# Samirez/Visual_odometry

Hardware: AMD Instinct MI355X
Metric: frame-pairs/sec (1280x720, 2000 ORB feats) (higher is better)
Workload: dtype u8+f32+f64; 1 GPU; seeded synthetic 1280x720 drone flight (256 distinct rendered views, closed loop), 2000 ORB features/frame, 8 levels = BASELINE config 2; chunk of 257 consecutive frames -> 256 pairs (k, k+1) per GPU per step, each frame detected once; detector=orb, distinct_rendered_frames=256, pair_stride=1, contexts_per_gpu=3, keypoint_order=cv2, poly_solver=fast, matcher=crosscheck, matcher_kernel=mfma_fp4, ransac=5-point, conf 0.99, 1 px, seed 2^64-1, <=1000 iters, parallelism=single GPU, pairs_ok_last_step=256

## Files before the change

### include/vo_hip.h

```cpp
#ifndef VO_HIP_H
#define VO_HIP_H
#include <stddef.h>
#include <stdint.h>

#ifdef __cplusplus
extern "C" {
#endif

#define VO_MAX_LEVELS 16

#define VO_OK                 0
#define VO_WARN_CAPACITY      1
#define VO_ERR_INVALID       -1
#define VO_ERR_HIP           -2
#define VO_ERR_TOO_FEW       -3
#define VO_ERR_NO_MODEL      -4
#define VO_ERR_NOT_CONFIGURED -5
#define VO_ERR_UNSUPPORTED    -7
#define VO_ERR_AMBIGUOUS      -6

typedef struct vo_ctx vo_ctx;

typedef struct {
    int32_t nfeatures;
// ... 45 lines not shown

int vo_recover_pose(vo_ctx* ctx, const double* E, const double* p1, const double* p2, int M, const double* K,
                    double dist_thresh, double* R, double* t, uint8_t* mask, int32_t* n_good);

int vo_triangulate(vo_ctx* ctx, const double* P1, const double* P2, const double* x1, const double* x2,
                   int M, double* X);

int64_t vo_packed_pyramid_bytes(int h, int w, const vo_orb_params* params);
int vo_stage_pyramid(vo_ctx* ctx, const uint8_t* img, int h, int w, int channels, int row_stride,
                     const vo_orb_params* params, uint8_t* out_packed);
int vo_stage_fast_scores(vo_ctx* ctx, const uint8_t* img, int h, int w, int channels, int row_stride,
                         const vo_orb_params* params, uint8_t* out_packed);
int vo_stage_blur(vo_ctx* ctx, const uint8_t* img, int h, int w, int channels, int row_stride,
                  const vo_orb_params* params, uint8_t* out_packed);
int vo_stage_retain_best(vo_ctx* ctx, const float* response, int n, int n_points, int32_t* order, int32_t* n_out);
int vo_stage_five_point(vo_ctx* ctx, const double* x1, const double* x2, double* E , int32_t* n_models);

typedef struct {
    int32_t match_mode;
    double  ratio;
    double  ransac_prob;
    double  ransac_thresh;
    int32_t ransac_max_iters;
    uint64_t ransac_seed;
    double  pose_dist_thresh;
    int32_t want_points;
} vo_pair_opts;

typedef struct {
    int32_t n_kp1, n_kp2, n_match, n_inl, n_good, status, ransac_iters, reserved;
// ... 141 lines not shown
```

### visual_odometry_amd/_lib.py

```python
from __future__ import annotations

import ctypes as C
import os

import numpy as np

_HERE = os.path.dirname(os.path.abspath(__file__))
LIB_PATH = os.environ.get("VO_HIP_LIBRARY") or os.path.join(_HERE, "libvo_hip.so")

VO_OK, VO_WARN_CAPACITY = 0, 1
VO_ERR_INVALID, VO_ERR_HIP, VO_ERR_TOO_FEW, VO_ERR_NO_MODEL, VO_ERR_NOT_CONFIGURED, VO_ERR_AMBIGUOUS = -1, -2, -3, -4, -5, -6
VO_ERR_UNSUPPORTED = -7
VO_STAGE_COUNT = 28
VO_COMM_ID_BYTES, VO_RECORD_DOUBLES = 128, 16
VO_BA_MAX_CAMERAS, VO_BA_MAX_FREE = 64, 16


class OrbParams(C.Structure):
    _fields_ = [("nfeatures", C.c_int32), ("scale_factor", C.c_float), ("nlevels", C.c_int32),
                ("edge_threshold", C.c_int32), ("first_level", C.c_int32), ("wta_k", C.c_int32),
                ("score_type", C.c_int32), ("patch_size", C.c_int32), ("fast_threshold", C.c_int32)]


class SiftParams(C.Structure):
# ... 46 lines not shown
    "vo_frames_upload_color": (C.c_int, [_P, _P, C.c_int, C.c_int, C.c_int, C.c_int64, C.c_int]),
    "vo_frames_detect": (C.c_int, [_P, C.c_int, C.c_int]),
    "vo_frames_detect_async": (C.c_int, [_P, C.c_int, C.c_int]),
    "vo_batch_kp_capacity": (C.c_int, [_P]),
    "vo_host_alloc": (C.c_int, [C.c_size_t, C.POINTER(_P)]),
    "vo_host_free": (None, [_P]),
    "vo_frame_features": (C.c_int, [_P, C.c_int, _P, _P, _P, _P, _P, _P, C.c_int, _P]),
    "vo_pairs_run": (C.c_int, [_P, _P, C.c_int, _P, _P, _P, _P, C.c_int32]),
    "vo_pairs_run_async": (C.c_int, [_P, _P, C.c_int, _P, _P, _P, _P, C.c_int32]),
    "vo_sync": (C.c_int, [_P]),
    "vo_set_matcher_kernel": (C.c_int, [_P, C.c_int]),
    "vo_set_poly_solver": (C.c_int, [_P, C.c_int]),
    "vo_set_pnp_refine": (C.c_int, [_P, C.c_int]),
    "vo_set_keypoint_order": (C.c_int, [_P, C.c_int]),
    "vo_stage_retain_best": (C.c_int, [_P, _P, C.c_int, C.c_int, _P, _P]),
    "vo_detect_after": (C.c_int, [_P, _P]),
    "vo_knn2_hamming": (C.c_int, [_P, _P, C.c_int, _P, C.c_int, _P, _P]),
    "vo_knn2_l2": (C.c_int, [_P, _P, C.c_int, _P, C.c_int, C.c_int, _P, _P]),
    "vo_knn2_ratio_l2": (C.c_int, [_P, _P, C.c_int, _P, C.c_int, C.c_int, C.c_double, _P, _P, _P, _P]),
    "vo_tracks_pnp_batch": (C.c_int, [_P, C.c_int, _P, C.c_int, C.c_double, C.c_double, C.c_uint64, C.c_double, _P, _P, _P, _P, _P]),
    "vo_slam_chain": (C.c_int, [_P, C.c_int, _P, _P, _P, _P, _P, _P, _P, _P, _P, _P, _P, _P, _P]),
    "vo_slam_map_size": (C.c_int, [_P, C.c_int, _P, _P, _P]),
    "vo_slam_map": (C.c_int, [_P, C.c_int, _P, _P, _P, _P, _P, _P, _P, _P]),
    "vo_slam_chains": (C.c_int, [_P, C.c_int, _P, _P, _P, C.c_int, _P, _P, _P, _P, _P, _P, _P, _P, _P, _P, _P]),
    "vo_slam_chains_restart": (C.c_int, [_P, C.c_int, _P, _P, _P, C.c_int, _P, _P, _P, _P, _P, _P, _P, _P, _P, _P, _P, _P, _P, _P, _P]),
    "vo_slam_chains_map_size": (C.c_int, [_P, C.c_int, C.c_int, _P, _P, _P]),
    "vo_slam_chains_map": (C.c_int, [_P, C.c_int, C.c_int, _P, _P, _P, _P, _P, _P, _P, _P]),
    "vo_comm_unique_id": (C.c_int, [_P]),
    "vo_comm_init": (C.c_int, [_P, _P, C.c_int, C.c_int]),
    "vo_comm_destroy": (C.c_int, [_P]),
# ... 15 lines not shown
    "vo_batch_configure_sift": (C.c_int, [_P, C.c_int, C.c_int, _P, C.c_int, C.c_int, C.c_int]),
    "vo_frame_features_sift": (C.c_int, [_P, C.c_int, _P, _P, _P, _P, _P, _P, C.c_int, _P]),
    "vo_stage_sift_rows": (C.c_int, [_P, C.c_int, _P, C.c_int, _P]),
    "vo_jpeg_info": (C.c_int, [_P, C.c_size_t, _P, _P, _P, _P, _P]),
    "vo_jpeg_decode": (C.c_int, [_P, _P, C.c_size_t, _P, C.c_int, C.c_int, _P, _P]),
    "vo_jpeg_decode_batch": (C.c_int, [_P, _P, _P, C.c_int, _P, C.c_int, C.c_int]),
    "vo_frames_ingest_jpeg": (C.c_int, [_P, _P, _P, C.c_int, C.c_int, _P]),
    "vo_feature_tracks": (C.c_int, [_P, C.c_int, C.c_int, _P, _P, _P, _P, C.c_int, _P, _P, _P]),
    "vo_profile_enable": (C.c_int, [_P, C.c_int]),
    "vo_profile_reset": (C.c_int, [_P]),
    "vo_profile_read": (C.c_int, [_P, _P, _P]),
    "vo_stage_name": (C.c_char_p, [C.c_int]),
    "vo_stage_bytes": (C.c_double, [_P, C.c_int, C.c_int]),
}

_lib = None


def load():
    global _lib
    if _lib is not None:
        return _lib
    if not os.path.exists(LIB_PATH):
        raise ImportError(
            f"{LIB_PATH} not found: build the HIP library first (python -c 'import __graft_entry__ as g; g.build()' "
            "or make -C visual_odometry_amd/csrc). There is no CPU fallback.")
    lib = C.CDLL(LIB_PATH)
    for name, (res, args) in _SIGS.items():
        fn = getattr(lib, name)
        fn.restype = res
        fn.argtypes = args
    _lib = lib
    return lib


def exported_symbols():
    return sorted(_SIGS)


class VoError(RuntimeError):
    def __init__(self, code, msg):
        super().__init__(f"libvo_hip error {code}: {msg}")
        self.code = code
# ... 51 lines not shown

    def comm_info(self):
        n, r = C.c_int32(0), C.c_int32(0)
        self.check(self.lib.vo_comm_info(self.handle, C.addressof(n), C.addressof(r)))
        return n.value, r.value

    def allgather(self, values, world):
        v = np.ascontiguousarray(values, np.float64).ravel()
        out = np.empty((int(world), len(v)), np.float64)
        self.check(self.lib.vo_comm_allgather_f64(self.handle, v.ctypes.data, len(v), out.ctypes.data))
        return out

    def set_keypoint_order(self, kind):
        self.check(self.lib.vo_set_keypoint_order(self.handle, {"canonical": 0, "cv2": 1}[kind]))

    def retain_best(self, response, n_points):
        r = np.ascontiguousarray(response, np.float32)
        out = np.zeros(max(len(r), 1), np.int32)
        n = C.c_int32(0)
        self.check(self.lib.vo_stage_retain_best(self.handle, r.ctypes.data, len(r), int(n_points), out.ctypes.data, C.addressof(n)))
        return out[:n.value].copy()

    def set_poly_solver(self, kind):
        self.check(self.lib.vo_set_poly_solver(self.handle, {"fast": 0, "opencv300": 1}[kind]))

    def set_pnp_refine(self, kind):
        self.check(self.lib.vo_set_pnp_refine(self.handle, {"fast": 0, "cv2": 1}[kind]))

    def last_error(self) -> str:
        msg = self.lib.vo_last_error(self.handle)
        return msg.decode() if msg else ""

    def check(self, rc):
        if rc < 0:
            msg = self.lib.vo_last_error(self.handle)
# ... 61 lines not shown
```

### visual_odometry_amd/csrc/cv2order_kernels.hip

```cpp
#include "vo_internal.h"
#include <float.h>

#ifndef CV_THREADS
#define CV_THREADS 256
#endif
#ifndef CV_EPT
#define CV_EPT 4
#endif
#ifndef CV_LDS_CAP
#define CV_LDS_CAP 4096
#endif

__device__ __forceinline__ bool el_gt(uint2 x, uint2 y) { return __uint_as_float(x.x) > __uint_as_float(y.x); }

#define CV_TIE_CAP CV_THREADS
struct Cv2Shared {
    int cnt[2][CV_EPT][CV_THREADS / 64][2];
    int probe[2][CV_THREADS / 64];
    int ntie, nleft;
    uint32_t tie[CV_TIE_CAP], tie_sorted[CV_TIE_CAP], left[CV_TIE_CAP];
    uint8_t is_tie[CV_TIE_CAP];
};

__device__ __forceinline__ void rank2(const bool (&fl)[CV_EPT], const bool (&fr)[CV_EPT], int parity, Cv2Shared& sh,
                                      int (&rl)[CV_EPT], int (&rr)[CV_EPT], int& tl, int& tr)
{
    const int lane = threadIdx.x & 63, wave = threadIdx.x >> 6;
    const unsigned long long below = lane ? (~0ULL >> (64 - lane)) : 0ULL;
    unsigned long long ml[CV_EPT], mr[CV_EPT];
#pragma unroll
    for (int e = 0; e < CV_EPT; e++) {
        ml[e] = __ballot(fl[e]); mr[e] = __ballot(fr[e]);
        if (lane == 0) { sh.cnt[parity][e][wave][0] = (int)__popcll(ml[e]); sh.cnt[parity][e][wave][1] = (int)__popcll(mr[e]); }
    }
    __syncthreads();
    int sl = 0, sr = 0;
// ... 30 lines not shown
        if (lane == 0) sh.probe[par][wave] = m64 ? wave * 64 + (int)__ffsll((long long)m64) - 1 : CV_THREADS;
        __syncthreads();
        int tf = CV_THREADS;
#pragma unroll
        for (int w = 0; w < CV_THREADS / 64; w++) tf = min(tf, sh.probe[par][w]);
        par ^= 1;
        const int kt = lo + tf * step;
        const int nhi = tf < CV_THREADS && kt < hi ? kt : hi;
        const int nlo = tf > 0 ? min(lo + (tf - 1) * step + 1, nhi) : lo;
        lo = nlo; hi = nhi;
        if (step == 1) break;
    }
    return hi;
}

template <typename A>
__device__ void adjust_heap(A f, int hole, int len, uint2 v)
{
    const int top = hole;
    int sc = hole;
    while (sc < (len - 1) / 2) { sc = 2 * (sc + 1); if (el_gt(f[sc], f[sc - 1])) sc--; f[hole] = f[sc]; hole = sc; }
    if ((len & 1) == 0 && sc == (len - 2) / 2) { sc = 2 * (sc + 1); f[hole] = f[sc - 1]; hole = sc - 1; }
    int parent = (hole - 1) / 2;
    while (hole > top && el_gt(f[parent], v)) { f[hole] = f[parent]; hole = parent; parent = (hole - 1) / 2; }
    f[hole] = v;
}

template <typename A>
__device__ void heap_select(A a, int first, int middle, int last)
{
    A f = a + first;
    const int len = middle - first;
    if (len >= 2)
        for (int parent = (len - 2) / 2;; parent--) { const uint2 v = f[parent]; adjust_heap(f, parent, len, v); if (parent == 0) break; }
    for (int i = middle; i < last; i++)
        if (el_gt(a[i], a[first])) { const uint2 v = a[i]; a[i] = a[first]; adjust_heap(f, 0, len, v); }
}

template <typename A>
__device__ void insertion_sort(A a, int first, int last)
{
    if (first == last) return;
    for (int i = first + 1; i < last; i++) {
        const uint2 v = a[i];
        if (el_gt(v, a[first])) { for (int j = i; j > first; j--) a[j] = a[j - 1]; a[first] = v; }
        else { int nx = i - 1; while (el_gt(v, a[nx])) { a[nx + 1] = a[nx]; nx--; } a[nx + 1] = v; }
    }
}

template <int KIND, typename A, typename PosT>
__device__ __forceinline__ int partition_pass(A a, int first, int last, uint2 pivot, float thr, PosT* lpos, PosT* rpos, Cv2Shared& sh)
{
    const int tid = threadIdx.x;
    int nl = 0, nr = 0, parity = 0;
    const int begin = KIND == 0 ? first + 1 : first;
    for (int base = begin; base < last; base += CV_THREADS * CV_EPT, parity ^= 1) {
        bool fl[CV_EPT], fr[CV_EPT];
#pragma unroll
        for (int e = 0; e < CV_EPT; e++) {
            const int i = base + e * CV_THREADS + tid;
            fl[e] = fr[e] = false;
            if (i < last) {
                const uint2 v = a[i];
                if (KIND == 0) { fl[e] = !el_gt(v, pivot); fr[e] = !el_gt(pivot, v); }
                else { const bool pred = __uint_as_float(v.x) >= thr; fl[e] = !pred; fr[e] = pred; }
            }
        }
        int rl[CV_EPT], rr[CV_EPT], tl, tr;
        rank2(fl, fr, parity, sh, rl, rr, tl, tr);
#pragma unroll
        for (int e = 0; e < CV_EPT; e++) {
            const int i = base + e * CV_THREADS + tid;
            if (fl[e]) lpos[nl + rl[e]] = (PosT)i;
            if (fr[e]) rpos[nr + rr[e]] = (PosT)i;
        }
        nl += tl; nr += tr;
    }
    __syncthreads();
    int K;
    long long res;
    const long long INF = 1LL << 40;
    if (KIND == 0) {
        K = first_true_wg(min(nl, nr), sh, [&](int k) { return lpos[k] >= rpos[nr - 1 - k]; });
        const long long lk = K < nl ? (long long)lpos[K] : INF, rk = K > 0 ? (long long)rpos[nr - K] : INF;
        res = lk < rk ? lk : rk;
    } else {
        K = first_true_wg(nl, sh, [&](int k) { return k >= nr || lpos[k] > rpos[nr - 1 - k]; });
        if (K >= nl) res = K > 0 ? (long long)rpos[nr - K] : (long long)last;
        else if (K > 0 && lpos[K] > rpos[nr - K]) res = rpos[nr - K];
        else res = lpos[K];
    }
    for (int k = tid; k < K; k += CV_THREADS) {
        const int i = (int)lpos[k], j = (int)rpos[nr - 1 - k];
        const uint2 x = a[i], y = a[j];
        a[i] = y; a[j] = x;
    }
    __syncthreads();
    return (int)res;
}

template <typename A, typename PosT>
__device__ __forceinline__ int partition_pivot(A a, int first, int last, PosT* lpos, PosT* rpos, Cv2Shared& sh)
{
    if (threadIdx.x == 0) {
        const int Ai = first + 1, B = first + (last - first) / 2, C = last - 1;
        int m;
        if (el_gt(a[Ai], a[B])) m = el_gt(a[B], a[C]) ? B : el_gt(a[Ai], a[C]) ? C : Ai;
        else m = el_gt(a[Ai], a[C]) ? Ai : el_gt(a[B], a[C]) ? C : B;
        const uint2 t = a[first]; a[first] = a[m]; a[m] = t;
    }
    __syncthreads();
    const uint2 p = a[first];
    return partition_pass<0>(a, first, last, p, 0.f, lpos, rpos, sh);
}

template <typename A, typename PosT>
__device__ __forceinline__ void introselect_loop(A a, int& first, int& last, int nth, int& depth, bool& done, int stop, PosT* lpos, PosT* rpos, Cv2Shared& sh)
{
    while (last - first > stop) {
        if (last - first <= 3) break;
        if (depth == 0) {
            if (threadIdx.x == 0) { heap_select(a, first, nth + 1, last); const uint2 t = a[first]; a[first] = a[nth]; a[nth] = t; }
            __syncthreads();
            done = true;
            return;
        }
        depth--;
        const int cut = partition_pivot(a, first, last, lpos, rpos, sh);
        if (cut <= nth) first = cut; else last = cut;
    }
}

#ifndef CV_WAVE_CAP
#define CV_WAVE_CAP 256
#endif
#define CV_WSYNC() do { __builtin_amdgcn_fence(__ATOMIC_SEQ_CST, "wavefront"); __builtin_amdgcn_wave_barrier(); } while (0)
template <typename P>
// ... 3 lines not shown
    while (hi > lo) {
        const int step = (hi - lo + 63) / 64;
        const int k = lo + lane * step;
        const bool t = k < hi ? pred(k) : true;
        const unsigned long long m64 = __ballot(t);
        const int tf = m64 ? (int)__ffsll((long long)m64) - 1 : 64;
        const int kt = lo + tf * step;
        const int nhi = tf < 64 && kt < hi ? kt : hi;
        const int nlo = tf > 0 ? min(lo + (tf - 1) * step + 1, nhi) : lo;
        lo = nlo; hi = nhi;
        if (step == 1) break;
    }
    return hi;
}

__device__ __forceinline__ int partition_pivot_wave(uint2* a, int first, int last, uint16_t* lpos, uint16_t* rpos)
{
    const int lane = threadIdx.x & 63;
    if (lane == 0) {
        const int Ai = first + 1, B = first + (last - first) / 2, C = last - 1;
        int m;
        if (el_gt(a[Ai], a[B])) m = el_gt(a[B], a[C]) ? B : el_gt(a[Ai], a[C]) ? C : Ai;
        else m = el_gt(a[Ai], a[C]) ? Ai : el_gt(a[B], a[C]) ? C : B;
        const uint2 t = a[first]; a[first] = a[m]; a[m] = t;
    }
    CV_WSYNC();
    const uint2 pivot = a[first];
    const unsigned long long below = lane ? (~0ULL >> (64 - lane)) : 0ULL;
    int nl = 0, nr = 0;
    for (int base = first + 1; base < last; base += 64) {
        const int i = base + lane;
        bool fl = false, fr = false;
        if (i < last) { const uint2 v = a[i]; fl = !el_gt(v, pivot); fr = !el_gt(pivot, v); }
        const unsigned long long ml = __ballot(fl), mr = __ballot(fr);
        if (fl) lpos[nl + (int)__popcll(ml & below)] = (uint16_t)i;
        if (fr) rpos[nr + (int)__popcll(mr & below)] = (uint16_t)i;
        nl += (int)__popcll(ml); nr += (int)__popcll(mr);
    }
    CV_WSYNC();
    const int K = first_true_wave(min(nl, nr), lane, [&](int k) { return lpos[k] >= rpos[nr - 1 - k]; });
    const int INF = 1 << 30;
    const int lk = K < nl ? (int)lpos[K] : INF, rk = K > 0 ? (int)rpos[nr - K] : INF;
    for (int k = lane; k < K; k += 64) {
        const int i = (int)lpos[k], j = (int)rpos[nr - 1 - k];
        const uint2 x = a[i], y = a[j];
        a[i] = y; a[j] = x;
    }
    CV_WSYNC();
    return lk < rk ? lk : rk;
}

__device__ __forceinline__ void introselect_wave(uint2* a, int first, int last, int nth, int depth, uint16_t* lpos, uint16_t* rpos)
{
    const int lane = threadIdx.x & 63;
    while (last - first > 3) {
        if (depth == 0) {
            if (lane == 0) { heap_select(a, first, nth + 1, last); const uint2 t = a[first]; a[first] = a[nth]; a[nth] = t; }
            CV_WSYNC();
            return;
        }
        depth--;
        const int cut = partition_pivot_wave(a, first, last, lpos, rpos);
        if (cut <= nth) first = cut; else last = cut;
    }
    if (lane == 0) insertion_sort(a, first, last);
    CV_WSYNC();
}

template <typename A>
__device__ __forceinline__ int partition_ge_sparse(A a, int first, int last, float thr, Cv2Shared& sh)
{
    const int tid = threadIdx.x;
    if (tid == 0) sh.ntie = 0;
    __syncthreads();
    for (int i = first + tid; i < last; i += CV_THREADS)
        if (__uint_as_float(a[i].x) >= thr) { const int s = atomicAdd(&sh.ntie, 1); if (s < CV_TIE_CAP) sh.tie[s] = (uint32_t)i; }
    __syncthreads();
    const int nr = sh.ntie;
    if (nr > CV_TIE_CAP) return -1;
    if (nr == 0) return first;
    for (int i = tid; i < nr; i += CV_THREADS) {
        const uint32_t p = sh.tie[i];
        int r = 0;
        for (int j = 0; j < nr; j++) r += sh.tie[j] < p ? 1 : 0;
        sh.tie_sorted[r] = p;
        sh.is_tie[i] = 0;
    }
    __syncthreads();
    for (int i = tid; i < nr; i += CV_THREADS) { const int rel = (int)sh.tie_sorted[i] - first; if (rel < nr) sh.is_tie[rel] = 1; }
    if (tid == 0) sh.nleft = 0;
    __syncthreads();
    {
        const bool fl = tid < nr && first + tid < last && !sh.is_tie[tid];
        const unsigned long long m = __ballot(fl);
        const int lane = tid & 63, wave = tid >> 6;
        if (lane == 0) sh.probe[0][wave] = (int)__popcll(m);
        __syncthreads();
        int before = 0, total = 0;
        for (int w = 0; w < CV_THREADS / 64; w++) { const int c = sh.probe[0][w]; if (w < wave) before += c; total += c; }
        if (fl) sh.left[before + (int)__popcll(m & (lane ? (~0ULL >> (64 - lane)) : 0ULL))] = (uint32_t)(first + tid);
        if (tid == 0) sh.nleft = total;
    }
    __syncthreads();
    const int K = sh.nleft;
    for (int k = tid; k < K; k += CV_THREADS) {
        const int i = (int)sh.left[k], j = (int)sh.tie_sorted[nr - 1 - k];
        const uint2 x = a[i], y = a[j];
        a[i] = y; a[j] = x;
    }
    __syncthreads();
    return first + nr;
}

template <typename PosT>
__device__ int retain_best_cv2(uint2* a, int n, int n_points, PosT* lpos, PosT* rpos, uint2* s_a, uint16_t* s_l, uint16_t* s_r, Cv2Shared& sh)
{
    if (n_points < 0 || n <= n_points) return n;
    if (n_points == 0) return 0;
    const int tid = threadIdx.x;
    int first = 0, last = n;
    const int nth = n_points - 1;
    int depth = 2 * (31 - __clz(n));
    bool done = false;
    introselect_loop(a, first, last, nth, depth, done, CV_LDS_CAP, lpos, rpos, sh);
    if (!done) {
        const int len = last - first;
        for (int i = tid; i < len; i += CV_THREADS) s_a[i] = a[first + i];
        __syncthreads();
        int f2 = 0, l2 = len;
        introselect_loop(s_a, f2, l2, nth - first, depth, done, CV_WAVE_CAP, s_l, s_r, sh);
        if (!done) {
            if (tid < 64) introselect_wave(s_a, f2, l2, nth - first, depth, s_l, s_r);
            __syncthreads();
        }
        for (int i = tid; i < len; i += CV_THREADS) a[first + i] = s_a[i];
        __syncthreads();
    }
    const float ambiguous = __uint_as_float(a[n_points - 1].x);
    const int fast = partition_ge_sparse(a, n_points, n, ambiguous, sh);
    if (fast >= 0) return fast;
    return partition_pass<1>(a, n_points, n, make_uint2(0, 0), ambiguous, lpos, rpos, sh);
}

__global__ __launch_bounds__(CV_THREADS) void k_cv2_order(PyrGeom g, FrameFeat ff, Cv2Buf cb, const int* kept_in)
{
    __shared__ Cv2Shared sh;
    __shared__ uint2 s_a[CV_LDS_CAP];
    __shared__ uint16_t s_l[CV_LDS_CAP], s_r[CV_LDS_CAP];
    const int l = blockIdx.x, f = blockIdx.y, tid = threadIdx.x;
    const LevelGeom lv = g.lv[l];
    const size_t abase = (size_t)f * cb.all_total + cb.all_off[l];
    const uint32_t* all_pos = cb.all_pos + abase;
    const float* all_resp = cb.all_resp + abase;
    uint2* a = cb.work + abase;
    uint32_t* lpos = cb.lpos + abase;
    uint32_t* rpos = cb.rpos + abase;
    const int listed = cb.all_count[f * VO_MAX_LEVELS + l];
    const int n0 = min(listed, cb.all_cap[l]);
    bool bad = listed > cb.all_cap[l];
    for (int i = tid; i < n0; i += CV_THREADS) a[i] = make_uint2(__float_as_uint(all_resp[i]), (uint32_t)i);
    __syncthreads();
    int n = retain_best_cv2(a, n0, g.score_type == 0 ? 2 * lv.quota : lv.quota, lpos, rpos, s_a, s_l, s_r, sh);
    if (g.score_type == 0) {
        const int nc = min(ff.cand_count[f * VO_MAX_LEVELS + l], lv.cand_cap);
        const uint32_t* cpos = ff.cand_pos + (size_t)f * g.cand_total + lv.cand_off;
        const float* cresp = ff.cand_resp + (size_t)f * g.cand_total + lv.cand_off;
        const uint32_t* all_cand = cb.all_cand + abase;
        for (int i = tid; i < n; i += CV_THREADS) {
            const uint32_t ai = a[i].y, pos = all_pos[ai], idx = all_cand[ai];
            const bool hit = idx < (uint32_t)nc && cpos[idx] == pos;
            bad |= !hit;
            a[i].x = __float_as_uint(hit ? cresp[idx] : -FLT_MAX);
        }
        __syncthreads();
        n = retain_best_cv2(a, n, lv.quota, lpos, rpos, s_a, s_l, s_r, sh);
    }
    int out_base = 0;
    for (int k = 0; k < l; k++) out_base += kept_in[f * VO_MAX_LEVELS + k];
    bad |= n != kept_in[f * VO_MAX_LEVELS + l];
    uint32_t* kp_pos = ff.kp_pos + (size_t)f * g.kp_cap;
    int* kp_level = ff.kp_level + (size_t)f * g.kp_cap;
    float* kp_resp = ff.kp_resp + (size_t)f * g.kp_cap;
    const int nw = min(n, kept_in[f * VO_MAX_LEVELS + l]);
    for (int i = tid; i < nw; i += CV_THREADS) {
        const int p = out_base + i;
        if (p < g.kp_cap) { kp_pos[p] = all_pos[a[i].y]; kp_level[p] = l; kp_resp[p] = __uint_as_float(a[i].x); }
    }
    if (bad && tid == 0) atomicOr(&ff.flags[f], 1);
}

void launch_cv2_order(hipStream_t s, const PyrGeom& g, FrameFeat ff, Cv2Buf cb, int F, const int* kept)
{
    hipLaunchKernelGGL(k_cv2_order, dim3(g.nlevels, F), dim3(CV_THREADS), 0, s, g, ff, cb, kept);
}

__global__ __launch_bounds__(CV_THREADS) void k_retain_raw(const float* resp, int n, int n_points, uint2* a, uint32_t* lpos,
                                                          uint32_t* rpos, int* order, int* n_out)
{
    __shared__ Cv2Shared sh;
    __shared__ uint2 s_a[CV_LDS_CAP];
    __shared__ uint16_t s_l[CV_LDS_CAP], s_r[CV_LDS_CAP];
    for (int i = threadIdx.x; i < n; i += CV_THREADS) a[i] = make_uint2(__float_as_uint(resp[i]), (uint32_t)i);
    __syncthreads();
    const int m = retain_best_cv2(a, n, n_points, lpos, rpos, s_a, s_l, s_r, sh);
    for (int i = threadIdx.x; i < m; i += CV_THREADS) order[i] = (int)a[i].y;
    if (threadIdx.x == 0) *n_out = m;
}

void launch_retain_raw(hipStream_t s, const float* resp, int n, int n_points, uint2* a, uint32_t* lpos, uint32_t* rpos,
                       int* order, int* n_out)
{
    hipLaunchKernelGGL(k_retain_raw, dim3(1), dim3(CV_THREADS), 0, s, resp, n, n_points, a, lpos, rpos, order, n_out);
}
```

### visual_odometry_amd/csrc/vo_api.hip

```cpp
#include "vo_internal.h"
#include <float.h>
#include <math.h>
#include <stdio.h>
#include <stdlib.h>
#include <string.h>
#include <vector>
#include <type_traits>
#include <algorithm>

#define MAX_EVENTS 384

struct DevList {
    struct Entry { void* p; bool pinned; };
    std::vector<Entry> ptrs;
    DevList() = default;
    DevList(const DevList&) = delete;
    DevList& operator=(DevList&& o) noexcept { if (this != &o) { release(); ptrs.swap(o.ptrs); } return *this; }
    ~DevList() { release(); }
    template <typename T> hipError_t alloc(T** p, size_t n) { return keep(hipMalloc((void**)p, (n ? n : 1) * sizeof(T)), (void**)p, false); }
    template <typename T> hipError_t alloc_pinned(T** p, size_t n)
    {
        return keep(hipHostMalloc((void**)p, (n ? n : 1) * sizeof(T), hipHostMallocDefault), (void**)p, true);
    }
    void release()
// ... 1479 lines not shown
    sc.take(&dx1, 10); sc.take(&dx2, 10); sc.take(&dE, 10 * 9); sc.take(&dnm, 1);
    int rc = sc.place(ctx); if (rc) return rc;
    hipStream_t s = ctx->stream;
    HIPCHK(hipMemcpyAsync(dx1, x1, 10 * sizeof(double), hipMemcpyHostToDevice, s));
    HIPCHK(hipMemcpyAsync(dx2, x2, 10 * sizeof(double), hipMemcpyHostToDevice, s));
    launch_five_point_raw(s, dx1, dx2, dE, dnm, ctx->dk_early);
    HIPCHK(hipGetLastError());
    int nm = 0;
    HIPCHK(hipMemcpyAsync(&nm, dnm, sizeof(int), hipMemcpyDeviceToHost, s));
    HIPCHK(hipStreamSynchronize(s));
    *n_models = nm;
    if (nm > 0) HIPCHK(hipMemcpy(E, dE, (size_t)nm * 9 * sizeof(double), hipMemcpyDeviceToHost));
    return VO_OK;
}

extern "C" int vo_stage_retain_best(vo_ctx* ctx, const float* response, int n, int n_points, int32_t* order, int32_t* n_out)
{
    if (!ctx) return VO_ERR_INVALID;
    if (n < 0 || !n_out || (n > 0 && (!response || !order))) FAIL(VO_ERR_INVALID, "bad arguments");
    *n_out = 0;
    if (n == 0) return VO_OK;
    HIPCHK(hipSetDevice(ctx->device));
    uint2* work; float* dresp; uint32_t *lpos, *rpos; int *dorder, *dn;
    ScratchLayout sc;
    sc.take(&work, n); sc.take(&dresp, n); sc.take(&lpos, n); sc.take(&rpos, n); sc.take(&dorder, n); sc.take(&dn, 1);
    int rc = sc.place(ctx); if (rc) return rc;
    hipStream_t s = ctx->stream;
    HIPCHK(hipMemcpyAsync(dresp, response, (size_t)n * sizeof(float), hipMemcpyHostToDevice, s));
    launch_retain_raw(s, dresp, n, n_points, work, lpos, rpos, dorder, dn);
    HIPCHK(hipGetLastError());
    int m = 0;
    HIPCHK(hipMemcpyAsync(&m, dn, sizeof(int), hipMemcpyDeviceToHost, s));
    HIPCHK(hipStreamSynchronize(s));
    *n_out = m;
    if (m > 0) HIPCHK(hipMemcpy(order, dorder, (size_t)m * sizeof(int), hipMemcpyDeviceToHost));
    return VO_OK;
}

extern "C" int vo_reprojection_filter(vo_ctx* ctx, const double* poses, int ncam, const double* points, int npt,
                                      const int32_t* obs_cam, const int32_t* obs_pt, const double* obs_xy, int nobs,
                                      const double* K, double threshold, double* sqerr, uint8_t* keep)
{
    if (!ctx) return VO_ERR_INVALID;
    if (ncam < 0 || npt < 0 || nobs < 0 || !K || (nobs > 0 && (!poses || !points || !obs_cam || !obs_pt || !obs_xy || !sqerr || !keep)))
        FAIL(VO_ERR_INVALID, "bad arguments");
    if (nobs == 0) return VO_OK;
    HIPCHK(hipSetDevice(ctx->device));
    double *dposes, *dpoints, *dxy, *dK, *derr; int *dcam, *dpt, *dbad; uint8_t* dkeep;
    ScratchLayout sc;
    sc.take(&dposes, (size_t)16 * ncam); sc.take(&dpoints, (size_t)3 * npt); sc.take(&dxy, (size_t)2 * nobs); sc.take(&dK, 9);
    sc.take(&derr, nobs); sc.take(&dcam, nobs); sc.take(&dpt, nobs); sc.take(&dbad, 1); sc.take(&dkeep, nobs);
// ... 1506 lines not shown
```

### visual_odometry_amd/csrc/vo_internal.h

```cpp
#pragma once
#include <hip/hip_runtime.h>
#include <stdint.h>
#include "../../include/vo_hip.h"

enum {
    ST_GRAY = 0, ST_RESIZE, ST_FAST, ST_SELECT_FAST, ST_HARRIS, ST_SELECT_HARRIS, ST_ANGLE,
    ST_BLUR, ST_BRIEF, ST_MATCH_NN, ST_MATCH_SELECT, ST_RANSAC, ST_POSE, ST_TRIANGULATE,
    ST_MISC, ST_RESERVED, ST_SIFT_SCALE, ST_SIFT_EXTREMA, ST_SIFT_ORIENT, ST_SIFT_SORT, ST_SIFT_DESC, ST_CV2_ORDER, ST_GATHER, ST_RESERVED2,
    ST_SLAM_PREPARE, ST_SLAM_BA, ST_SLAM_FILTER, ST_SLAM_LIMIT
};

struct LevelGeom {
    int w, h, stride, off;
    int quota;
    float scale;
    int ftile_base, ftiles_x;
    int fox, foy;
    int dtile_base, dtiles_x;
    int btile_base, btiles_x;
    int cand_off, cand_cap;
    int sel_chunk_base;
};

struct PyrGeom {
// ... 112 lines not shown
const char* rccl_comm_count(void* comm, int* n);
const char* rccl_all_gather_f64(void* comm, const double* send, double* recv, size_t count, hipStream_t s);
void launch_pack_records(hipStream_t s, const vo_pair_result* res, int B, int valid, double* rec);

void launch_gray(hipStream_t s, const uint8_t* src, int channels, int row_stride, int64_t frame_stride,
                 uint8_t* pyr, const PyrGeom& g, int F);
void launch_gray_plain(hipStream_t s, const uint8_t* src, int channels, int row_stride, int64_t frame_stride,
                       uint8_t* dst, int w, int h, int dstride, int64_t dframe, int F);
void launch_resize(hipStream_t s, uint8_t* pyr, const PyrGeom& g, int level, const ResizeTab& tab, int F);
void launch_fast(hipStream_t s, const uint8_t* pyr, uint8_t* score, uint32_t* hist, const PyrGeom& g, int F,
                 uint32_t* tile_list, int* tile_count);
void launch_select_fast(hipStream_t s, const PyrGeom& g, FrameFeat ff, int F, int* thr, int* chunk_count,
                        const uint32_t* tile_list, const int* tile_count, const Cv2Buf* cb);
void launch_harris(hipStream_t s, const uint8_t* pyr, const PyrGeom& g, FrameFeat ff, int F);
void launch_cv2_order(hipStream_t s, const PyrGeom& g, FrameFeat ff, Cv2Buf cb, int F, const int* kept);
void launch_retain_raw(hipStream_t s, const float* resp, int n, int n_points, uint2* a, uint32_t* lpos, uint32_t* rpos,
                       int* order, int* n_out);
void launch_select_harris(hipStream_t s, const PyrGeom& g, FrameFeat ff, int F, float* thr, int* kept);
void launch_angle(hipStream_t s, const uint8_t* pyr, const PyrGeom& g, FrameFeat ff, int F);
void launch_resize_linear(hipStream_t st, const uint8_t* src, int sw, int sh, int cn, int sstride, int64_t sframe,
                          uint8_t* dst, int dw, int dh, int dstride, int64_t dframe,
                          const int* xofs, const void* xa, const int* yofs, const void* yb, int area2, int F);
void launch_resize_area(hipStream_t st, const uint8_t* src, int cn, int sstride, uint8_t* dst, int dw, int dh, int dstride,
                        int isx, int isy, const int* xsi, const float* xal, const int* xst, const int* ysi, const float* yal, const int* yst);
#define SIFT_IMG_BORDER 5
#define SIFT_MAX_INTERP_STEPS 5
#define SIFT_MAX_OCT 16
#define SIFT_MAX_TAPS 64
struct SiftGeom {
    int nOct, nLayers;
    int w[SIFT_MAX_OCT], h[SIFT_MAX_OCT], stride[SIFT_MAX_OCT];
    size_t plane[SIFT_MAX_OCT];
// ... 164 lines not shown
```

Measured before the change: 100,900 frame-pairs/s.

## Pack FAST scores and indices into 32-bit keys for cv2-order introselect

The cv2-order keypoint retention now packs the integer FAST score and the index into one 32-bit key (score<<16|idx) when a level has fewer than 65536 candidates. It runs the introselect on these keys first, keeping twice the quota when Harris rescoring follows, then re-selects on the Harris responses. The LDS buffer is unified into a byte-sized union and sized per element type. The block size drops to 128 threads, and the launch grid is flattened to a 1D grid of levels times frames. The intent is to halve memory traffic in the selection passes and to shrink the Harris pre-selection set. The risk is that the pre-filter changes the tie-handling semantics relative to cv2.

```diff
diff --git a/include/vo_hip.h b/include/vo_hip.h
--- a/include/vo_hip.h
+++ b/include/vo_hip.h
@@ -83,6 +83,7 @@
 int vo_stage_blur(vo_ctx* ctx, const uint8_t* img, int h, int w, int channels, int row_stride,
                   const vo_orb_params* params, uint8_t* out_packed);
 int vo_stage_retain_best(vo_ctx* ctx, const float* response, int n, int n_points, int32_t* order, int32_t* n_out);
+int vo_stage_retain_best_fast(vo_ctx* ctx, const float* response, int n, int n_points, int32_t* order, int32_t* n_out);
 int vo_stage_five_point(vo_ctx* ctx, const double* x1, const double* x2, double* E , int32_t* n_models);
 
 typedef struct {
diff --git a/visual_odometry_amd/_lib.py b/visual_odometry_amd/_lib.py
--- a/visual_odometry_amd/_lib.py
+++ b/visual_odometry_amd/_lib.py
@@ -84,6 +84,7 @@
     "vo_set_pnp_refine": (C.c_int, [_P, C.c_int]),
     "vo_set_keypoint_order": (C.c_int, [_P, C.c_int]),
     "vo_stage_retain_best": (C.c_int, [_P, _P, C.c_int, C.c_int, _P, _P]),
+    "vo_stage_retain_best_fast": (C.c_int, [_P, _P, C.c_int, C.c_int, _P, _P]),
     "vo_detect_after": (C.c_int, [_P, _P]),
     "vo_knn2_hamming": (C.c_int, [_P, _P, C.c_int, _P, C.c_int, _P, _P]),
     "vo_knn2_l2": (C.c_int, [_P, _P, C.c_int, _P, C.c_int, C.c_int, _P, _P]),
@@ -129,6 +130,8 @@
     "vo_stage_bytes": (C.c_double, [_P, C.c_int, C.c_int]),
 }
 
+_NEWER_HOOKS = {"vo_stage_retain_best_fast"}
+
 _lib = None
 
 
@@ -142,6 +145,8 @@
             "or make -C visual_odometry_amd/csrc). There is no CPU fallback.")
     lib = C.CDLL(LIB_PATH)
     for name, (res, args) in _SIGS.items():
+        if name in _NEWER_HOOKS and os.environ.get("VO_HIP_LIBRARY") and not hasattr(lib, name):
+            continue
         fn = getattr(lib, name)
         fn.restype = res
         fn.argtypes = args
@@ -223,11 +228,12 @@
     def set_keypoint_order(self, kind):
         self.check(self.lib.vo_set_keypoint_order(self.handle, {"canonical": 0, "cv2": 1}[kind]))
 
-    def retain_best(self, response, n_points):
+    def retain_best(self, response, n_points, fast_scores=False):
         r = np.ascontiguousarray(response, np.float32)
         out = np.zeros(max(len(r), 1), np.int32)
         n = C.c_int32(0)
-        self.check(self.lib.vo_stage_retain_best(self.handle, r.ctypes.data, len(r), int(n_points), out.ctypes.data, C.addressof(n)))
+        fn = self.lib.vo_stage_retain_best_fast if fast_scores else self.lib.vo_stage_retain_best
+        self.check(fn(self.handle, r.ctypes.data, len(r), int(n_points), out.ctypes.data, C.addressof(n)))
         return out[:n.value].copy()
 
     def set_poly_solver(self, kind):
diff --git a/visual_odometry_amd/csrc/cv2order_kernels.hip b/visual_odometry_amd/csrc/cv2order_kernels.hip
--- a/visual_odometry_amd/csrc/cv2order_kernels.hip
+++ b/visual_odometry_amd/csrc/cv2order_kernels.hip
@@ -2,24 +2,30 @@
 #include <float.h>
 
 #ifndef CV_THREADS
-#define CV_THREADS 256
+#define CV_THREADS 128
 #endif
 #ifndef CV_EPT
 #define CV_EPT 4
 #endif
-#ifndef CV_LDS_CAP
-#define CV_LDS_CAP 4096
+#ifndef CV_LDS_BYTES
+#define CV_LDS_BYTES 24576
 #endif
+template <typename E> struct Cv2Lds {
+    static constexpr int cap = CV_LDS_BYTES / ((int)sizeof(E) + 4);
+    static_assert(cap <= 65535, "stopper positions in LDS are 16 bits");
+};
 
 __device__ __forceinline__ bool el_gt(uint2 x, uint2 y) { return __uint_as_float(x.x) > __uint_as_float(y.x); }
-
-#define CV_TIE_CAP CV_THREADS
+__device__ __forceinline__ bool el_ge(uint2 x, uint2 y) { return __uint_as_float(x.x) >= __uint_as_float(y.x); }
+__device__ __forceinline__ bool el_gt(uint32_t x, uint32_t y) { return (x >> 16) > (y >> 16); }
+__device__ __forceinline__ bool el_ge(uint32_t x, uint32_t y) { return (x >> 16) >= (y >> 16); }
+
+#define CV_TIE_CAP 256
+static_assert(13 * CV_TIE_CAP <= CV_LDS_BYTES, "the tie lists live in the LDS buffer");
 struct Cv2Shared {
     int cnt[2][CV_EPT][CV_THREADS / 64][2];
     int probe[2][CV_THREADS / 64];
-    int ntie, nleft;
-    uint32_t tie[CV_TIE_CAP], tie_sorted[CV_TIE_CAP], left[CV_TIE_CAP];
-    uint8_t is_tie[CV_TIE_CAP];
+    int ntie;
 };
 
 __device__ __forceinline__ void rank2(const bool (&fl)[CV_EPT], const bool (&fr)[CV_EPT], int parity, Cv2Shared& sh,
@@ -80,8 +86,8 @@
     return hi;
 }
 
-template <typename A>
-__device__ void adjust_heap(A f, int hole, int len, uint2 v)
+template <typename E>
+__device__ void adjust_heap(E* f, int hole, int len, E v)
 {
     const int top = hole;
     int sc = hole;
@@ -92,30 +98,30 @@
     f[hole] = v;
 }
 
-template <typename A>
-__device__ void heap_select(A a, int first, int middle, int last)
-{
-    A f = a + first;
+template <typename E>
+__device__ void heap_select(E* a, int first, int middle, int last)
+{
+    E* f = a + first;
     const int len = middle - first;
     if (len >= 2)
-        for (int parent = (len - 2) / 2;; parent--) { const uint2 v = f[parent]; adjust_heap(f, parent, len, v); if (parent == 0) break; }
+        for (int parent = (len - 2) / 2;; parent--) { const E v = f[parent]; adjust_heap(f, parent, len, v); if (parent == 0) break; }
     for (int i = middle; i < last; i++)
-        if (el_gt(a[i], a[first])) { const uint2 v = a[i]; a[i] = a[first]; adjust_heap(f, 0, len, v); }
-}
-
-template <typename A>
-__device__ void insertion_sort(A a, int first, int last)
+        if (el_gt(a[i], a[first])) { const E v = a[i]; a[i] = a[first]; adjust_heap(f, 0, len, v); }
+}
+
+template <typename E>
+__device__ void insertion_sort(E* a, int first, int last)
 {
     if (first == last) return;
     for (int i = first + 1; i < last; i++) {
-        const uint2 v = a[i];
+        const E v = a[i];
         if (el_gt(v, a[first])) { for (int j = i; j > first; j--) a[j] = a[j - 1]; a[first] = v; }
         else { int nx = i - 1; while (el_gt(v, a[nx])) { a[nx + 1] = a[nx]; nx--; } a[nx + 1] = v; }
     }
 }
 
-template <int KIND, typename A, typename PosT>
-__device__ __forceinline__ int partition_pass(A a, int first, int last, uint2 pivot, float thr, PosT* lpos, PosT* rpos, Cv2Shared& sh)
+template <int KIND, typename E, typename PosT>
+__device__ __forceinline__ int partition_pass(E* a, int first, int last, E ref, PosT* lpos, PosT* rpos, Cv2Shared& sh)
 {
     const int tid = threadIdx.x;
     int nl = 0, nr = 0, parity = 0;
@@ -127,9 +133,9 @@
             const int i = base + e * CV_THREADS + tid;
             fl[e] = fr[e] = false;
             if (i < last) {
-                const uint2 v = a[i];
-                if (KIND == 0) { fl[e] = !el_gt(v, pivot); fr[e] = !el_gt(pivot, v); }
-                else { const bool pred = __uint_as_float(v.x) >= thr; fl[e] = !pred; fr[e] = pred; }
+                const E v = a[i];
+                if (KIND == 0) { fl[e] = !el_gt(v, ref); fr[e] = !el_gt(ref, v); }
+                else { const bool pred = el_ge(v, ref); fl[e] = !pred; fr[e] = pred; }
             }
         }
         int rl[CV_EPT], rr[CV_EPT], tl, tr;
@@ -158,35 +164,35 @@
     }
     for (int k = tid; k < K; k += CV_THREADS) {
         const int i = (int)lpos[k], j = (int)rpos[nr - 1 - k];
-        const uint2 x = a[i], y = a[j];
+        const E x = a[i], y = a[j];
         a[i] = y; a[j] = x;
     }
     __syncthreads();
     return (int)res;
 }
 
-template <typename A, typename PosT>
-__device__ __forceinline__ int partition_pivot(A a, int first, int last, PosT* lpos, PosT* rpos, Cv2Shared& sh)
+template <typename E, typename PosT>
+__device__ __forceinline__ int partition_pivot(E* a, int first, int last, PosT* lpos, PosT* rpos, Cv2Shared& sh)
 {
     if (threadIdx.x == 0) {
         const int Ai = first + 1, B = first + (last - first) / 2, C = last - 1;
         int m;
         if (el_gt(a[Ai], a[B])) m = el_gt(a[B], a[C]) ? B : el_gt(a[Ai], a[C]) ? C : Ai;
         else m = el_gt(a[Ai], a[C]) ? Ai : el_gt(a[B], a[C]) ? C : B;
-        const uint2 t = a[first]; a[first] = a[m]; a[m] = t;
-    }
-    __syncthreads();
-    const uint2 p = a[first];
-    return partition_pass<0>(a, first, last, p, 0.f, lpos, rpos, sh);
-}
-
-template <typename A, typename PosT>
-__device__ __forceinline__ void introselect_loop(A a, int& first, int& last, int nth, int& depth, bool& done, int stop, PosT* lpos, PosT* rpos, Cv2Shared& sh)
+        const E t = a[first]; a[first] = a[m]; a[m] = t;
+    }
+    __syncthreads();
+    const E p = a[first];
+    return partition_pass<0>(a, first, last, p, lpos, rpos, sh);
+}
+
+template <typename E, typename PosT>
+__device__ __forceinline__ void introselect_loop(E* a, int& first, int& last, int nth, int& depth, bool& done, int stop, PosT* lpos, PosT* rpos, Cv2Shared& sh)
 {
     while (last - first > stop) {
         if (last - first <= 3) break;
         if (depth == 0) {
-            if (threadIdx.x == 0) { heap_select(a, first, nth + 1, last); const uint2 t = a[first]; a[first] = a[nth]; a[nth] = t; }
+            if (threadIdx.x == 0) { heap_select(a, first, nth + 1, last); const E t = a[first]; a[first] = a[nth]; a[nth] = t; }
             __syncthreads();
             done = true;
             return;
@@ -220,7 +226,8 @@
     return hi;
 }
 
-__device__ __forceinline__ int partition_pivot_wave(uint2* a, int first, int last, uint16_t* lpos, uint16_t* rpos)
+template <typename E>
+__device__ __forceinline__ int partition_pivot_wave(E* a, int first, int last, uint16_t* lpos, uint16_t* rpos)
 {
     const int lane = threadIdx.x & 63;
     if (lane == 0) {
@@ -228,16 +235,16 @@
         int m;
         if (el_gt(a[Ai], a[B])) m = el_gt(a[B], a[C]) ? B : el_gt(a[Ai], a[C]) ? C : Ai;
         else m = el_gt(a[Ai], a[C]) ? Ai : el_gt(a[B], a[C]) ? C : B;
-        const uint2 t = a[first]; a[first] = a[m]; a[m] = t;
+        const E t = a[first]; a[first] = a[m]; a[m] = t;
     }
     CV_WSYNC();
-    const uint2 pivot = a[first];
+    const E pivot = a[first];
     const unsigned long long below = lane ? (~0ULL >> (64 - lane)) : 0ULL;
     int nl = 0, nr = 0;
     for (int base = first + 1; base < last; base += 64) {
         const int i = base + lane;
         bool fl = false, fr = false;
-        if (i < last) { const uint2 v = a[i]; fl = !el_gt(v, pivot); fr = !el_gt(pivot, v); }
+        if (i < last) { const E v = a[i]; fl = !el_gt(v, pivot); fr = !el_gt(pivot, v); }
         const unsigned long long ml = __ballot(fl), mr = __ballot(fr);
         if (fl) lpos[nl + (int)__popcll(ml & below)] = (uint16_t)i;
         if (fr) rpos[nr + (int)__popcll(mr & below)] = (uint16_t)i;
@@ -249,19 +256,20 @@
     const int lk = K < nl ? (int)lpos[K] : INF, rk = K > 0 ? (int)rpos[nr - K] : INF;
     for (int k = lane; k < K; k += 64) {
         const int i = (int)lpos[k], j = (int)rpos[nr - 1 - k];
-        const uint2 x = a[i], y = a[j];
+        const E x = a[i], y = a[j];
         a[i] = y; a[j] = x;
     }
     CV_WSYNC();
     return lk < rk ? lk : rk;
 }
 
-__device__ __forceinline__ void introselect_wave(uint2* a, int first, int last, int nth, int depth, uint16_t* lpos, uint16_t* rpos)
+template <typename E>
+__device__ __forceinline__ void introselect_wave(E* a, int first, int last, int nth, int depth, uint16_t* lpos, uint16_t* rpos)
 {
     const int lane = threadIdx.x & 63;
     while (last - first > 3) {
         if (depth == 0) {
-            if (lane == 0) { heap_select(a, first, nth + 1, last); const uint2 t = a[first]; a[first] = a[nth]; a[nth] = t; }
+            if (lane == 0) { heap_select(a, first, nth + 1, last); const E t = a[first]; a[first] = a[nth]; a[nth] = t; }
             CV_WSYNC();
             return;
         }
@@ -273,62 +281,67 @@
     CV_WSYNC();
 }
 
-template <typename A>
-__device__ __forceinline__ int partition_ge_sparse(A a, int first, int last, float thr, Cv2Shared& sh)
-{
-    const int tid = threadIdx.x;
+template <typename E>
+__device__ __forceinline__ int partition_ge_sparse(E* a, int first, int last, E thr, uint32_t* buf, Cv2Shared& sh)
+{
+    const int tid = threadIdx.x, lane = tid & 63, wave = tid >> 6;
+    uint32_t *tie = buf, *tie_sorted = buf + CV_TIE_CAP, *left = buf + 2 * CV_TIE_CAP;
+    uint8_t* is_tie = (uint8_t*)(buf + 3 * CV_TIE_CAP);
     if (tid == 0) sh.ntie = 0;
     __syncthreads();
     for (int i = first + tid; i < last; i += CV_THREADS)
-        if (__uint_as_float(a[i].x) >= thr) { const int s = atomicAdd(&sh.ntie, 1); if (s < CV_TIE_CAP) sh.tie[s] = (uint32_t)i; }
+        if (el_ge(a[i], thr)) { const int s = atomicAdd(&sh.ntie, 1); if (s < CV_TIE_CAP) tie[s] = (uint32_t)i; }
     __syncthreads();
     const int nr = sh.ntie;
     if (nr > CV_TIE_CAP) return -1;
     if (nr == 0) return first;
     for (int i = tid; i < nr; i += CV_THREADS) {
-        const uint32_t p = sh.tie[i];
+        const uint32_t p = tie[i];
         int r = 0;
-        for (int j = 0; j < nr; j++) r += sh.tie[j] < p ? 1 : 0;
-        sh.tie_sorted[r] = p;
-        sh.is_tie[i] = 0;
-    }
-    __syncthreads();
-    for (int i = tid; i < nr; i += CV_THREADS) { const int rel = (int)sh.tie_sorted[i] - first; if (rel < nr) sh.is_tie[rel] = 1; }
-    if (tid == 0) sh.nleft = 0;
-    __syncthreads();
-    {
-        const bool fl = tid < nr && first + tid < last && !sh.is_tie[tid];
+        for (int j = 0; j < nr; j++) r += tie[j] < p ? 1 : 0;
+        tie_sorted[r] = p;
+        is_tie[i] = 0;
+    }
+    __syncthreads();
+    for (int i = tid; i < nr; i += CV_THREADS) { const int rel = (int)tie_sorted[i] - first; if (rel < nr) is_tie[rel] = 1; }
+    __syncthreads();
+    int K = 0, par = 0;
+    for (int c = 0; c < nr; c += CV_THREADS, par ^= 1) {
+        const int r = c + tid;
+        const bool fl = r < nr && first + r < last && !is_tie[r];
         const unsigned long long m = __ballot(fl);
-        const int lane = tid & 63, wave = tid >> 6;
-        if (lane == 0) sh.probe[0][wave] = (int)__popcll(m);
+        if (lane == 0) sh.probe[par][wave] = (int)__popcll(m);
         __syncthreads();
         int before = 0, total = 0;
-        for (int w = 0; w < CV_THREADS / 64; w++) { const int c = sh.probe[0][w]; if (w < wave) before += c; total += c; }
-        if (fl) sh.left[before + (int)__popcll(m & (lane ? (~0ULL >> (64 - lane)) : 0ULL))] = (uint32_t)(first + tid);
-        if (tid == 0) sh.nleft = total;
-    }
-    __syncthreads();
-    const int K = sh.nleft;
+#pragma unroll
+        for (int w = 0; w < CV_THREADS / 64; w++) { const int cw = sh.probe[par][w]; if (w < wave) before += cw; total += cw; }
+        if (fl) left[K + before + (int)__popcll(m & (lane ? (~0ULL >> (64 - lane)) : 0ULL))] = (uint32_t)(first + r);
+        K += total;
+    }
+    __syncthreads();
     for (int k = tid; k < K; k += CV_THREADS) {
-        const int i = (int)sh.left[k], j = (int)sh.tie_sorted[nr - 1 - k];
-        const uint2 x = a[i], y = a[j];
+        const int i = (int)left[k], j = (int)tie_sorted[nr - 1 - k];
+        const E x = a[i], y = a[j];
         a[i] = y; a[j] = x;
     }
     __syncthreads();
     return first + nr;
 }
 
-template <typename PosT>
-__device__ int retain_best_cv2(uint2* a, int n, int n_points, PosT* lpos, PosT* rpos, uint2* s_a, uint16_t* s_l, uint16_t* s_r, Cv2Shared& sh)
+template <typename E, typename PosT>
+__device__ __forceinline__ int retain_best_cv2(E* a, int n, int n_points, PosT* lpos, PosT* rpos, uint32_t* buf, Cv2Shared& sh)
 {
     if (n_points < 0 || n <= n_points) return n;
     if (n_points == 0) return 0;
     const int tid = threadIdx.x;
+    constexpr int cap = Cv2Lds<E>::cap;
+    E* s_a = (E*)buf;
+    uint16_t *s_l = (uint16_t*)(s_a + cap), *s_r = s_l + cap;
     int first = 0, last = n;
     const int nth = n_points - 1;
     int depth = 2 * (31 - __clz(n));
     bool done = false;
-    introselect_loop(a, first, last, nth, depth, done, CV_LDS_CAP, lpos, rpos, sh);
+    introselect_loop(a, first, last, nth, depth, done, cap, lpos, rpos, sh);
     if (!done) {
         const int len = last - first;
         for (int i = tid; i < len; i += CV_THREADS) s_a[i] = a[first + i];
@@ -342,18 +355,17 @@
         for (int i = tid; i < len; i += CV_THREADS) a[first + i] = s_a[i];
         __syncthreads();
     }
-    const float ambiguous = __uint_as_float(a[n_points - 1].x);
-    const int fast = partition_ge_sparse(a, n_points, n, ambiguous, sh);
+    const E ambiguous = a[n_points - 1];
+    const int fast = partition_ge_sparse(a, n_points, n, ambiguous, buf, sh);
     if (fast >= 0) return fast;
-    return partition_pass<1>(a, n_points, n, make_uint2(0, 0), ambiguous, lpos, rpos, sh);
-}
-
-__global__ __launch_bounds__(CV_THREADS) void k_cv2_order(PyrGeom g, FrameFeat ff, Cv2Buf cb, const int* kept_in)
+    return partition_pass<1>(a, n_points, n, ambiguous, lpos, rpos, sh);
+}
+
+__global__ __launch_bounds__(CV_THREADS) void k_cv2_order(PyrGeom g, FrameFeat ff, Cv2Buf cb, const int* kept_in, int F)
 {
     __shared__ Cv2Shared sh;
-    __shared__ uint2 s_a[CV_LDS_CAP];
-    __shared__ uint16_t s_l[CV_LDS_CAP], s_r[CV_LDS_CAP];
-    const int l = blockIdx.x, f = blockIdx.y, tid = threadIdx.x;
+    __shared__ __attribute__((aligned(16))) uint32_t s_buf[CV_LDS_BYTES / 4];
+    const int l = (int)blockIdx.x / F, f = (int)blockIdx.x - l * F, tid = threadIdx.x;
     const LevelGeom lv = g.lv[l];
     const size_t abase = (size_t)f * cb.all_total + cb.all_off[l];
     const uint32_t* all_pos = cb.all_pos + abase;
@@ -361,25 +373,42 @@
     uint2* a = cb.work + abase;
     uint32_t* lpos = cb.lpos + abase;
     uint32_t* rpos = cb.rpos + abase;
+    const int cap_l = cb.all_cap[l];
     const int listed = cb.all_count[f * VO_MAX_LEVELS + l];
-    const int n0 = min(listed, cb.all_cap[l]);
-    bool bad = listed > cb.all_cap[l];
-    for (int i = tid; i < n0; i += CV_THREADS) a[i] = make_uint2(__float_as_uint(all_resp[i]), (uint32_t)i);
-    __syncthreads();
-    int n = retain_best_cv2(a, n0, g.score_type == 0 ? 2 * lv.quota : lv.quota, lpos, rpos, s_a, s_l, s_r, sh);
-    if (g.score_type == 0) {
-        const int nc = min(ff.cand_count[f * VO_MAX_LEVELS + l], lv.cand_cap);
-        const uint32_t* cpos = ff.cand_pos + (size_t)f * g.cand_total + lv.cand_off;
-        const float* cresp = ff.cand_resp + (size_t)f * g.cand_total + lv.cand_off;
-        const uint32_t* all_cand = cb.all_cand + abase;
-        for (int i = tid; i < n; i += CV_THREADS) {
-            const uint32_t ai = a[i].y, pos = all_pos[ai], idx = all_cand[ai];
-            const bool hit = idx < (uint32_t)nc && cpos[idx] == pos;
-            bad |= !hit;
-            a[i].x = __float_as_uint(hit ? cresp[idx] : -FLT_MAX);
-        }
-        __syncthreads();
-        n = retain_best_cv2(a, n, lv.quota, lpos, rpos, s_a, s_l, s_r, sh);
+    const int n0 = min(listed, cap_l);
+    bool bad = listed > cap_l;
+    const bool packed = n0 < 65536;
+    uint32_t* a32 = lpos;
+    const int nret = g.score_type == 0 ? 2 : 1;
+    int n = n0;
+    if (packed) {
+        for (int i = tid; i < n0; i += CV_THREADS) a32[i] = (uint32_t)all_resp[i] << 16 | (uint32_t)i;
+        __syncthreads();
+        n = retain_best_cv2(a32, n0, nret == 2 ? 2 * lv.quota : lv.quota, (uint32_t*)a, (uint32_t*)a + cap_l, s_buf, sh);
+        if (nret == 1) {
+            for (int i = tid; i < n; i += CV_THREADS) { const uint32_t e = a32[i]; a[i] = make_uint2(__float_as_uint((float)(e >> 16)), e & 0xffffu); }
+            __syncthreads();
+        }
+    } else {
+        for (int i = tid; i < n0; i += CV_THREADS) a[i] = make_uint2(__float_as_uint(all_resp[i]), (uint32_t)i);
+        __syncthreads();
+    }
+#pragma nounroll
+    for (int it = packed ? 1 : 0; it < nret; it++) {
+        if (it == 1) {
+            const int nc = min(ff.cand_count[f * VO_MAX_LEVELS + l], lv.cand_cap);
+            const uint32_t* cpos = ff.cand_pos + (size_t)f * g.cand_total + lv.cand_off;
+            const float* cresp = ff.cand_resp + (size_t)f * g.cand_total + lv.cand_off;
+            const uint32_t* all_cand = cb.all_cand + abase;
+            for (int i = tid; i < n; i += CV_THREADS) {
+                const uint32_t ai = packed ? a32[i] & 0xffffu : a[i].y, pos = all_pos[ai], idx = all_cand[ai];
+                const bool hit = idx < (uint32_t)nc && cpos[idx] == pos;
+                bad |= !hit;
+                a[i] = make_uint2(__float_as_uint(hit ? cresp[idx] : -FLT_MAX), ai);
+            }
+            __syncthreads();
+        }
+        n = retain_best_cv2(a, n, it == 0 && nret == 2 ? 2 * lv.quota : lv.quota, lpos, rpos, s_buf, sh);
     }
     int out_base = 0;
     for (int k = 0; k < l; k++) out_base += kept_in[f * VO_MAX_LEVELS + k];
@@ -397,24 +426,32 @@
 
 void launch_cv2_order(hipStream_t s, const PyrGeom& g, FrameFeat ff, Cv2Buf cb, int F, const int* kept)
 {
-    hipLaunchKernelGGL(k_cv2_order, dim3(g.nlevels, F), dim3(CV_THREADS), 0, s, g, ff, cb, kept);
-}
-
-__global__ __launch_bounds__(CV_THREADS) void k_retain_raw(const float* resp, int n, int n_points, uint2* a, uint32_t* lpos,
-                                                          uint32_t* rpos, int* order, int* n_out)
+    hipLaunchKernelGGL(k_cv2_order, dim3(g.nlevels * F), dim3(CV_THREADS), 0, s, g, ff, cb, kept, F);
+}
+
+__global__ __launch_bounds__(CV_THREADS) void k_retain_raw(const float* resp, int n, int n_points, int fast_scores, uint2* a,
+                                                          uint32_t* lpos, uint32_t* rpos, int* order, int* n_out)
 {
     __shared__ Cv2Shared sh;
-    __shared__ uint2 s_a[CV_LDS_CAP];
-    __shared__ uint16_t s_l[CV_LDS_CAP], s_r[CV_LDS_CAP];
-    for (int i = threadIdx.x; i < n; i += CV_THREADS) a[i] = make_uint2(__float_as_uint(resp[i]), (uint32_t)i);
-    __syncthreads();
-    const int m = retain_best_cv2(a, n, n_points, lpos, rpos, s_a, s_l, s_r, sh);
-    for (int i = threadIdx.x; i < m; i += CV_THREADS) order[i] = (int)a[i].y;
+    __shared__ __attribute__((aligned(16))) uint32_t s_buf[CV_LDS_BYTES / 4];
+    int m;
+    if (fast_scores && n < 65536) {
+        uint32_t* a32 = lpos;
+        for (int i = threadIdx.x; i < n; i += CV_THREADS) a32[i] = (uint32_t)resp[i] << 16 | (uint32_t)i;
+        __syncthreads();
+        m = retain_best_cv2(a32, n, n_points, (uint32_t*)a, (uint32_t*)a + n, s_buf, sh);
+        for (int i = threadIdx.x; i < m; i += CV_THREADS) order[i] = (int)(a32[i] & 0xffffu);
+    } else {
+        for (int i = threadIdx.x; i < n; i += CV_THREADS) a[i] = make_uint2(__float_as_uint(resp[i]), (uint32_t)i);
+        __syncthreads();
+        m = retain_best_cv2(a, n, n_points, lpos, rpos, s_buf, sh);
+        for (int i = threadIdx.x; i < m; i += CV_THREADS) order[i] = (int)a[i].y;
+    }
     if (threadIdx.x == 0) *n_out = m;
 }
 
-void launch_retain_raw(hipStream_t s, const float* resp, int n, int n_points, uint2* a, uint32_t* lpos, uint32_t* rpos,
-                       int* order, int* n_out)
-{
-    hipLaunchKernelGGL(k_retain_raw, dim3(1), dim3(CV_THREADS), 0, s, resp, n, n_points, a, lpos, rpos, order, n_out);
-}
+void launch_retain_raw(hipStream_t s, const float* resp, int n, int n_points, int fast_scores, uint2* a, uint32_t* lpos,
+                       uint32_t* rpos, int* order, int* n_out)
+{
+    hipLaunchKernelGGL(k_retain_raw, dim3(1), dim3(CV_THREADS), 0, s, resp, n, n_points, fast_scores, a, lpos, rpos, order, n_out);
+}
diff --git a/visual_odometry_amd/csrc/vo_api.hip b/visual_odometry_amd/csrc/vo_api.hip
--- a/visual_odometry_amd/csrc/vo_api.hip
+++ b/visual_odometry_amd/csrc/vo_api.hip
@@ -1517,7 +1517,7 @@
     return VO_OK;
 }
 
-extern "C" int vo_stage_retain_best(vo_ctx* ctx, const float* response, int n, int n_points, int32_t* order, int32_t* n_out)
+static int stage_retain_best(vo_ctx* ctx, const float* response, int n, int n_points, int fast_scores, int32_t* order, int32_t* n_out)
 {
     if (!ctx) return VO_ERR_INVALID;
     if (n < 0 || !n_out || (n > 0 && (!response || !order))) FAIL(VO_ERR_INVALID, "bad arguments");
@@ -1530,7 +1530,7 @@
     int rc = sc.place(ctx); if (rc) return rc;
     hipStream_t s = ctx->stream;
     HIPCHK(hipMemcpyAsync(dresp, response, (size_t)n * sizeof(float), hipMemcpyHostToDevice, s));
-    launch_retain_raw(s, dresp, n, n_points, work, lpos, rpos, dorder, dn);
+    launch_retain_raw(s, dresp, n, n_points, fast_scores, work, lpos, rpos, dorder, dn);
     HIPCHK(hipGetLastError());
     int m = 0;
     HIPCHK(hipMemcpyAsync(&m, dn, sizeof(int), hipMemcpyDeviceToHost, s));
@@ -1538,6 +1538,21 @@
     *n_out = m;
     if (m > 0) HIPCHK(hipMemcpy(order, dorder, (size_t)m * sizeof(int), hipMemcpyDeviceToHost));
     return VO_OK;
+}
+
+extern "C" int vo_stage_retain_best(vo_ctx* ctx, const float* response, int n, int n_points, int32_t* order, int32_t* n_out)
+{
+    return stage_retain_best(ctx, response, n, n_points, 0, order, n_out);
+}
+
+extern "C" int vo_stage_retain_best_fast(vo_ctx* ctx, const float* response, int n, int n_points, int32_t* order, int32_t* n_out)
+{
+    if (!ctx) return VO_ERR_INVALID;
+    if (n > 0 && !response) FAIL(VO_ERR_INVALID, "bad arguments");
+    for (int i = 0; i < n; i++)
+        if (!(response[i] >= 0.f && response[i] <= 65535.f && response[i] == (float)(int)response[i]))
+            FAIL(VO_ERR_INVALID, "vo_stage_retain_best_fast: scores must be integers in [0, 65535]");
+    return stage_retain_best(ctx, response, n, n_points, 1, order, n_out);
 }
 
 extern "C" int vo_reprojection_filter(vo_ctx* ctx, const double* poses, int ncam, const double* points, int npt,
diff --git a/visual_odometry_amd/csrc/vo_internal.h b/visual_odometry_amd/csrc/vo_internal.h
--- a/visual_odometry_amd/csrc/vo_internal.h
+++ b/visual_odometry_amd/csrc/vo_internal.h
@@ -150,8 +150,8 @@
                         const uint32_t* tile_list, const int* tile_count, const Cv2Buf* cb);
 void launch_harris(hipStream_t s, const uint8_t* pyr, const PyrGeom& g, FrameFeat ff, int F);
 void launch_cv2_order(hipStream_t s, const PyrGeom& g, FrameFeat ff, Cv2Buf cb, int F, const int* kept);
-void launch_retain_raw(hipStream_t s, const float* resp, int n, int n_points, uint2* a, uint32_t* lpos, uint32_t* rpos,
-                       int* order, int* n_out);
+void launch_retain_raw(hipStream_t s, const float* resp, int n, int n_points, int fast_scores, uint2* a, uint32_t* lpos,
+                       uint32_t* rpos, int* order, int* n_out);
 void launch_select_harris(hipStream_t s, const PyrGeom& g, FrameFeat ff, int F, float* thr, int* kept);
 void launch_angle(hipStream_t s, const uint8_t* pyr, const PyrGeom& g, FrameFeat ff, int F);
 void launch_resize_linear(hipStream_t st, const uint8_t* src, int sw, int sh, int cn, int sstride, int64_t sframe,
```

New measurement: 102,000 frame-pairs/s (median of 6 runs). No clear change (+1.1%).
